# ArmastusChen/Learning-Continuous-Implicit-Representation-for-Near-Periodic-Patterns

Measured on AMD Instinct MI355X. Metric: fitted pixels/sec/GPU (512^2 grid, 256-wide MLP) + iters-to-target-PSNR, higher is better.
Workload: dtype bf16

## Files before the change

learning-continuous-implicit-representation-for-near-periodic-patterns_amd/csrc/npp_api.hip:

```cpp
#include <math.h>
#include <stdarg.h>
#include <stdio.h>
#include <string.h>
#include <vector>

#include "npp_common.h"

namespace npp {

static thread_local char g_err[512] = "";

void set_error(const char* fmt, ...) {
  va_list ap;
  va_start(ap, fmt);
  vsnprintf(g_err, sizeof(g_err), fmt, ap);
  va_end(ap);
}

int check_launch(const char* what) {
  hipError_t e = hipGetLastError();
  if (e != hipSuccess) {
    set_error("%s: %s", what, hipGetErrorString(e));
    return NPP_ERR_LAUNCH;
  }
// ... 190 lines not shown
#pragma unroll
  for (int e = 0; e < 4; ++e) {
    if (e < cnt) {
      if (n < d.n_out[l]) {
        const __bf16 w = (__bf16)pn[e];
        if (!fwd4) {
          const int64_t pf = fwd_pack_pos(d, l, n, k);
          if (pf >= 0) a.wf[pf] = w;
        }
        const int64_t pb = bwd_pack_pos(b, l, n, k);
        if (pb >= 0) a.wb[pb] = w;
      }
      if (++k == d.n_in[l]) { k = 0; ++n; }
      if (n >= d.n_out[l] && i + e + 1 >= d.b_off[l] + d.n_out[l]) {
        do { ++l; } while (l < kNumLayers && !d.present[l]);
        if (l >= kNumLayers) break;
        n = 0; k = 0;
      }
    }
  }
}

static uint16_t f32_to_bf16_host(float f) {
  uint32_t u;
  memcpy(&u, &f, 4);
  if ((u & 0x7fffffffu) > 0x7f800000u) return (uint16_t)((u >> 16) | 0x40);
  u += 0x7FFF + ((u >> 16) & 1);
  return (uint16_t)(u >> 16);
}

__global__ void selftest_kernel(float* out) {
  const int lane = threadIdx.x & 63;
  const int m = lane & 31, h = lane >> 5;
  bf16x8 a, b;
#pragma unroll
  for (int j = 0; j < 8; ++j) {
    const int k = 8 * h + j;
    a[j] = (__bf16)(float)(((m * 3 + k * 5) % 5) - 2);
    b[j] = (__bf16)(float)(((k * 7 + m * 2) % 4) - 1);
  }
  f32x16 acc = {};
  acc = mfma_bf16(a, b, acc);
#pragma unroll
  for (int r = 0; r < 16; ++r) out[acc_row(r, h) * 32 + m] = acc[r];
  f32x16 y = {};
#pragma unroll
  for (int s = 0; s < 2; ++s) {
    bf16x8 x = pack_acc(acc, s), a2;
#pragma unroll
    for (int j = 0; j < 8; ++j) {
      const int k = 16 * s + perm16(h, j);
      a2[j] = (__bf16)(float)(((m * 5 + k * 3) % 7) - 3);
    }
    y = mfma_bf16(a2, x, y);
  }
#pragma unroll
  for (int r = 0; r < 16; ++r) out[1024 + acc_row(r, h) * 32 + m] = y[r];

  __shared__ __attribute__((aligned(16))) char tile[16384];
  for (int u = lane; u < 1024; u += 64) {
    const int hh = u & 1, b = (u >> 1) & 31, bt = (u >> 6) & 1, ks = u >> 7;
    bf16x8 f;
#pragma unroll
    for (int j = 0; j < 8; ++j) {
      const int feat = 16 * ks + perm16(hh, j), row = bt * 32 + b;
      f[j] = (__bf16)(float)(((7 * feat + 3 * row) % 251) - 125);
    }
    *(bf16x8*)(tile + wfmt_unit(8, 0, ks, bt, b, hh)) = f;
  }
  __syncthreads();
  for (int tt = 0; tt < 4; ++tt)
    for (int t = 0; t < 4; ++t) {
      const bf16x8 f = wfrag_read(tile, wfrag_offset(tt, t, lane));
#pragma unroll
      for (int j = 0; j < 8; ++j) out[2048 + ((tt * 4 + t) * 64 + lane) * 8 + j] = (float)f[j];
    }
}

static int tune_env(const char* name, int dflt) {
  const char* e = getenv(name);
  return e && *e ? atoi(e) : dflt;
}
Tunables g_tune = {tune_env("NPP_CONV_WINK", 1), tune_env("NPP_CONV_WIN", 1), tune_env("NPP_CONV_WSTAT", 1), tune_env("NPP_CONV_PAIR", 15),
                   tune_env("NPP_LIGHT_DET", 1), tune_env("NPP_STASH8", 1)};

}

using namespace npp;

extern "C" {

int npp_version(void) { return 100; }

int npp_tune(const char* key, int value) {
  struct { const char* k; int* v; } tab[] = {{"conv_wink", &g_tune.conv_wink}, {"conv_win", &g_tune.conv_win},
                                             {"conv_wstat", &g_tune.conv_wstat}, {"conv_pair", &g_tune.conv_pair},
                                             {"stash8", &g_tune.stash8}, {"light_det", &g_tune.light_det}};
  if (key)
    for (auto& t : tab)
      if (!strcmp(key, t.k)) {
        const int old = __atomic_load_n(t.v, __ATOMIC_RELAXED);
        if (value >= 0) __atomic_store_n(t.v, value, __ATOMIC_RELAXED);
        return old;
      }
  set_error("npp_tune: unknown key '%s'", key ? key : "(null)");
  return NPP_ERR_ARG;
}
const char* npp_last_error_string(void) { return g_err; }

int npp_device_count(void) {
  int n = 0;
  hipError_t e = hipGetDeviceCount(&n);
  if (e != hipSuccess) {
    set_error("hipGetDeviceCount: %s", hipGetErrorString(e));
    (void)hipGetLastError();
    return 0;
  }
  return n;
}

static int check_kw(int K, int width) {
  if (K < 1 || K > NPP_MAX_K) { set_error("K=%d outside [1,%d]", K, NPP_MAX_K); return NPP_ERR_ARG; }
  if (width != NPP_WIDTH) {
    set_error("width=%d: this build is specialised for width %d", width, NPP_WIDTH);
    return NPP_ERR_UNSUPPORTED;
  }
  return NPP_OK;
}

int npp_param_layout(int K, int width, const char** names, int64_t* offsets, int32_t* rows,
                     int32_t* cols, int64_t* total) {
  int rc = check_kw(K, width);
  if (rc) return rc;
  const NetDesc d = make_desc(K);
  int n = 0;
  for (int l = 0; l < kNumLayers; ++l) {
    if (!d.present[l]) continue;
    for (int wb = 0; wb < 2; ++wb) {
      snprintf(g_name_buf[n], sizeof(g_name_buf[n]), "%s.%s", kNames[l], wb ? "bias" : "weight");
      if (names) names[n] = g_name_buf[n];
      if (offsets) offsets[n] = wb ? d.b_off[l] : d.w_off[l];
      if (rows) rows[n] = d.n_out[l];
      if (cols) cols[n] = wb ? 1 : d.n_in[l];
      ++n;
    }
  }
  if (total) *total = d.total_params;
  return n;
}

int64_t npp_pack_bytes(int K, int width, int which) {
  if (check_kw(K, width)) return -1;
  return 16 * (which == 0 ? make_desc(K).wf_total16 : bwd_total16(K));
}

int npp_pack_weights(const float* d_params, void* d_wf, void* d_wb, int K, int width, void* stream) {
  int rc = check_kw(K, width);
  if (rc) return rc;
  if (!d_params || !d_wf || !d_wb) { set_error("npp_pack_weights: null pointer"); return NPP_ERR_ARG; }
  const NetDesc d = make_desc(K);
  const BwdDesc b = make_bwd_desc(K);
  const int64_t nf = d.wf_total16, nb = bwd_total16(K);
  const int threads = 256;
  const int64_t blocks = (nf + nb + threads - 1) / threads;
  hipLaunchKernelGGL(pack_weights_kernel, dim3((unsigned)blocks), dim3(threads), 0, (hipStream_t)stream,
                     d_params, (bf16x8*)d_wf, (bf16x8*)d_wb, d, b, nf, nb);
  return check_launch("npp_pack_weights");
}

int npp_pack_weights_host(const float* params, void* wf, void* wb, int K, int width) {
  int rc = check_kw(K, width);
  if (rc) return rc;
  const NetDesc d = make_desc(K);
  const BwdDesc b = make_bwd_desc(K);
  uint16_t* f = (uint16_t*)wf;
  uint16_t* g = (uint16_t*)wb;
  for (int64_t u = 0; u < d.wf_total16; ++u) {
    int l, ks, nt, lane;
    if (!fwd_unit(d, u, l, ks, nt, lane)) { set_error("fwd unit %lld unmapped", (long long)u); return NPP_ERR_ARG; }
// ... 162 lines not shown
```

learning-continuous-implicit-representation-for-near-periodic-patterns_amd/csrc/npp_common.h:

```cpp
#pragma once
#include <hip/hip_runtime.h>
#include <stdint.h>
#include "npp_layout.h"

typedef __attribute__((ext_vector_type(8))) __bf16 bf16x8;
typedef __attribute__((ext_vector_type(4))) __bf16 bf16x4;
typedef __attribute__((ext_vector_type(2))) __bf16 bf16x2;
typedef __attribute__((ext_vector_type(16))) float f32x16;
typedef __attribute__((ext_vector_type(4))) float f32x4;
typedef __attribute__((ext_vector_type(2))) float f32x2;
typedef __attribute__((ext_vector_type(4))) uint32_t u32x4;
typedef __attribute__((ext_vector_type(8))) _Float16 f16x8;

namespace npp {

void set_error(const char* fmt, ...);
int check_launch(const char* what);
struct SmemOnce { unsigned long long done = 0; };

struct Tunables {
  int conv_wink;
  int conv_win;
  int conv_wstat;
  int conv_pair;
  int light_det;
  int stash8;
};
extern Tunables g_tune;
bool smem_attr(SmemOnce& once, const void* fn, int bytes);

constexpr float kInv2Pi = 0.15915494309189535f;

struct EmbedDev {
  int32_t K, H, W, pad;
  float inv_w, inv_h;
  float cs[NPP_MAX_K][2], sn[NPP_MAX_K][2];
  float per[NPP_MAX_K][2][NPP_N_OFF];
  float freq[NPP_N_FREQ];
  float freq_rev[NPP_N_FREQ];
};

__device__ __forceinline__ float sincos_pi2(float x, bool want_cos) {
  const float jf = rintf(x * 0.636619772367581343f);
  float y = fmaf(-jf, 1.5703125f, x);
  y = fmaf(-jf, 4.837512969970703125e-4f, y);
  y = fmaf(-jf, 7.54978995489188e-8f, y);
  const int q = ((int)jf + (want_cos ? 1 : 0)) & 3;
  const float z = y * y;
  const float s = fmaf(y * z, fmaf(z, fmaf(z, -1.9515295891e-4f, 8.3321608736e-3f), -1.6666654611e-1f), y);
  const float c = fmaf(z * z, fmaf(z, fmaf(z, 2.443315711809948e-5f, -1.388731625493765e-3f), 4.166664568298827e-2f),
                       fmaf(z, -0.5f, 1.0f));
  const float r = (q & 1) ? c : s;
  return (q & 2) ? -r : r;
}

template <bool PRECISE>
__device__ __forceinline__ float warp_value(const EmbedDev& e, int p, int i, float y, float x) {
  const int ori = i >= 11;
  const int ii = ori ? i - 11 : i;
  if (ii == 0) {
    return ori ? (y / (float)e.H - 0.5f) * 2.0f : (x / (float)e.W - 0.5f) * 2.0f;
  }
  const int o = (ii - 1) >> 1;
  const bool is_cos = (ii - 1) & 1;
  const float per = e.per[p][ori][o];
  const float t = __fadd_rn(__fmul_rn(y, e.cs[p][ori]), __fmul_rn(x, e.sn[p][ori]));
  if (PRECISE) {
    float r = fmodf(t, per);
    if (r != 0.0f && ((per < 0.0f) != (r < 0.0f))) r += per;
    const float phi = ((r / per) * 2.0f) * 3.14159265358979323846f;
    return sincos_pi2(phi, is_cos);
  } else {
    const float q = floorf(t / per);
    float r = fmaf(-q, per, t);
    r = r < 0.0f ? r + per : r;
    r = r >= per ? r - per : r;
    const float rev = r / per;
    return is_cos ? __builtin_amdgcn_cosf(rev) : __builtin_amdgcn_sinf(rev);
  }
}

enum CoordMode { kCoordI32 = 0, kCoordF32 = 1, kCoordGrid = 2 };

__device__ __forceinline__ void grid_coord(const npp_grid& g, int64_t r, float& y, float& x) {
  const int64_t p = g.start + (r < g.n ? r : g.n - 1);
  const int64_t i = p / g.width;
  const int32_t j = (int32_t)(p - i * g.width);
  y = __fadd_rn(g.y0, __fdiv_rn((float)i, g.sy));
  x = __fadd_rn(g.x0, __fdiv_rn((float)j, g.sx));
}

template <int CM>
__device__ __forceinline__ void load_coord(const void* coords, const npp_grid& g, int64_t r, float& y, float& x) {
  if (CM == kCoordGrid) {
    grid_coord(g, r, y, x);
  } else if (CM == kCoordF32) {
    const float2 c = ((const float2*)coords)[r];
    y = c.x;
    x = c.y;
  } else {
    const int2 c = ((const int2*)coords)[r];
    y = (float)c.x;
    x = (float)c.y;
  }
}

__device__ __forceinline__ void sincos_pi2_both(float x, float& sn, float& cs) {
  const float jf = rintf(x * 0.636619772367581343f);
  float y = fmaf(-jf, 1.5703125f, x);
// ... 435 lines not shown
```

learning-continuous-implicit-representation-for-near-periodic-patterns_amd/csrc/npp_conv.hip:

```cpp
#include <stdlib.h>
#include <string.h>
#include <type_traits>

#include "npp_common.h"
#include "npp_trunk_layout.h"
#ifdef NPP_DIAG
#include "npp_diag.h"
#else
#define NPP_DIAG_FIELD
#define NPP_DIAG_FILL(a) do { } while (0)
#define NPP_STAMP(a, k) do { } while (0)
#define NPP_STAMP_DRAIN() do { } while (0)
#endif

namespace npp {

#ifndef NPP_CONV_RING
#define NPP_CONV_RING 9
#endif
constexpr int kConvRing = NPP_CONV_RING;
static_assert(kConvRing == 3 || kConvRing == 9, "ring depth");

enum ConvMode : int { kConvFwd = 0, kConvDgradMask = 1, kConvDgradLin = 2, kConvFwdPool = 3, kConvDgradPool = 4 };

// ... 567 lines not shown
    if (has_next) gload(ci + KG, st);
    const char* bA = gbase + buf * kBuf;
    const char* bW = bA + kA + h * wu * 16;
    frag_t A[2][CT], B[2][NPT];
    auto lread = [&](int set, int tap) {
      const int shift = (tap / 3) * a.Wp + (tap % 3);
#pragma unroll
      for (int ct = 0; ct < CT; ++ct) A[set][ct] = *(const frag_t*)(bA + ((ct * 9 + tap) * 64 + lane) * 16);
#pragma unroll
      for (int pt = 0; pt < NPT; ++pt) B[set][pt] = *(const frag_t*)(bW + (posw + 32 * pt + shift) * 16);
    };
    lread(0, 0);
#pragma unroll
    for (int tap = 0; tap < 9; ++tap) {
      if (tap + 1 < 9) lread((tap + 1) & 1, tap + 1);
#pragma unroll
      for (int ct = 0; ct < CT; ++ct)
#pragma unroll
        for (int pt = 0; pt < NPT; ++pt) acc[ct][pt] = mfma16(A[tap & 1][ct], B[tap & 1][pt], acc[ct][pt]);
    }
    if (has_next) sstore(buf ^ 1, st);
    __syncthreads();
    buf ^= 1;
  }
  NPP_STAMP(a, 3);
  float* red = (float*)klds;
  if (KG > 1) {
#pragma unroll
    for (int t = 0; t < NT; ++t) {
      if (t % KG == kg) continue;
#pragma unroll
      for (int r = 0; r < 16; ++r) red[(((pw * KG + kg) * NT + t) * 16 + r) * 64 + lane] = acc[t / NPT][t % NPT][r];
    }
    __syncthreads();
  }
#pragma unroll
  for (int t = 0; t < NT; ++t) {
    if (t % KG != kg) continue;
    const int q = t / KG, ct = t / NPT, pt = t % NPT;
    f32x16 v;
#pragma unroll
    for (int r = 0; r < 16; ++r) v[r] = 0.0f;
#pragma unroll
    for (int g = 0; g < KG; ++g) {
      if (g == kg) {
#pragma unroll
        for (int r = 0; r < 16; ++r) v[r] += acc[ct][pt][r];
      } else {
#pragma unroll
        for (int r = 0; r < 16; ++r) v[r] += red[(((pw * KG + g) * NT + t) * 16 + r) * 64 + lane];
      }
    }
    const int64_t p = (int64_t)(tile0 + NPT * pw + pt) * 32 + b;
    const int n = (int)((uint32_t)p / (uint32_t)a.S);
    const int r0 = (int)(p - (int64_t)n * a.S);
    const int yy = r0 / a.Wp, xx = r0 - yy * a.Wp;
    const bool interior = p < a.npos_valid && yy >= 1 && yy <= a.H && xx >= 1 && xx <= a.W;
    const int64_t tap_base = (((int64_t)n * a.Ctap) * a.H + (yy - 1)) * a.W + (xx - 1);
    const int cot = cot0 + ct;
#pragma unroll
    for (int s = 0; s < 2; ++s) {
      const int chunk = 4 * cot + 2 * s + h;
      if (chunk >= a.cout_chunks) continue;
      const int64_t unit = (int64_t)chunk * a.nposp + kConvGuard + p;
      frag_t o;
#pragma unroll
      for (int j = 0; j < 8; ++j) {
        const int co = 32 * cot + acc_row(8 * s + j, h);
        float x = v[8 * s + j];
        if (FWD) x = fminf(fmaxf(x + bias_r[q][8 * s + j], 0.0f), 65504.0f);
        if (MODE == kConvDgradMask) x = (float)gate[q][s][j] > 0.0f ? x : 0.0f;
        x = interior ? x : 0.0f;
        o[j] = (elem_t)x;
        if (a.tap && interior && co < a.Ctap)
          a.tap[tap_base + (int64_t)co * a.H * a.W] = a.has_scale ? x * a.tap_scale[co & 3] : x;
      }
      if (a.y) ((frag_t*)a.y)[unit] = o;
    }
  }
  NPP_STAMP(a, 4);
  NPP_STAMP_DRAIN();
  NPP_STAMP(a, 5);
  asm volatile("" :: "v"(pf_val));
}

__global__ void conv_pack_kernel(const float* __restrict__ w, int Cin, int Cout, int in_natural, int CIp ,
                                 f16x8* __restrict__ pf, int64_t nf, bf16x8* __restrict__ pb, int64_t nbk) {
  const int64_t u = (int64_t)blockIdx.x * blockDim.x + threadIdx.x;
  if (u < nf) {
    const int lane = (int)(u & 63);
    int64_t r = u >> 6;
    const int tap = (int)(r % 9); r /= 9;
    const int CI = CIp / 16;
    const int ci_step = (int)(r % CI);
    const int cot = (int)(r / CI);
    const int m = lane & 31, h = lane >> 5, co = 32 * cot + m;
    f16x8 o;
#pragma unroll
    for (int j = 0; j < 8; ++j) {
      const int c8 = 2 * ci_step + h;
      const int ci = in_natural ? c8 * 8 + j : conv_chan(c8, j);
      const float v = (co < Cout && ci < Cin) ? w[((int64_t)co * Cin + ci) * 9 + tap] : 0.0f;
      o[j] = (_Float16)fminf(fmaxf(v, -65504.0f), 65504.0f);
    }
    pf[u] = o;
  } else if (u < nf + nbk) {
    const int64_t ub = u - nf;
    const int lane = (int)(ub & 63);
    int64_t r = ub >> 6;
    const int tap = (int)(r % 9); r /= 9;
    const int CO = Cout / 16;
    const int co_step = (int)(r % CO);
    const int cit = (int)(r / CO);
    const int m = lane & 31, h = lane >> 5, ci = 32 * cit + m;
    bf16x8 o;
#pragma unroll
    for (int j = 0; j < 8; ++j) {
      const int co = conv_chan(2 * co_step + h, j);
      const float v = (ci < Cin && co < Cout) ? w[((int64_t)co * Cin + ci) * 9 + (8 - tap)] : 0.0f;
      o[j] = (__bf16)v;
    }
    pb[ub] = o;
  }
}

__global__ void trunk_image_in_kernel(const float* __restrict__ img, int N, int H, int W, float s0, float s1, float s2,
                                      float b0, float b1, float b2, f16x8* __restrict__ out, int64_t nposp,
                                      int64_t npos_round) {
  const int64_t p = (int64_t)blockIdx.x * blockDim.x + threadIdx.x;
  if (p >= npos_round) return;
  const int Wp = W + 2, S = (H + 2) * Wp;
  const int n = (int)(p / S), r = (int)(p - (int64_t)n * S), y = r / Wp, x = r - y * Wp;
  f16x8 o;
#pragma unroll
  for (int j = 0; j < 8; ++j) o[j] = (_Float16)0.0f;
  const f16x8 z = o;
  if (n < N && y >= 1 && y <= H && x >= 1 && x <= W) {
    const int64_t base = ((int64_t)n * 3 * H + (y - 1)) * W + (x - 1);
    const int64_t cs = (int64_t)H * W;
    o[0] = trunk_in_f16(img[base], s0, b0);
    o[1] = trunk_in_f16(img[base + cs], s1, b1);
    o[2] = trunk_in_f16(img[base + 2 * cs], s2, b2);
  }
  out[kConvGuard + p] = o;
  out[nposp + kConvGuard + p] = z;
}

__global__ void trunk_patch_in_kernel(const float* __restrict__ pred, const float* __restrict__ fake,
                                      const float* __restrict__ fmask, const float* __restrict__ real,
                                      const float* __restrict__ rmask, int n_p, int k, int P, int comp, float s0, float s1,
                                      float s2, float b0, float b1, float b2, f16x8* __restrict__ out, int64_t nposp,
                                      int64_t npos_round, float* __restrict__ xy, float* __restrict__ zero, int n_zero,
                                      int which, PixelLossArgs pl, int nb_loss) {
  if ((int)blockIdx.x < nb_loss) {
    pixel_loss_body(pl, (int)blockIdx.x, nb_loss);
    return;
  }
  const int64_t p = (int64_t)((int)blockIdx.x - nb_loss) * blockDim.x + threadIdx.x;
  if (p < n_zero) zero[p] = 0.0f;
  if (p >= npos_round) return;
  const int Wp = P + 2, S = (P + 2) * Wp, nk = n_p * k;
  const int nl = (int)(p / S), r = (int)(p - (int64_t)nl * S), y = r / Wp, x = r - y * Wp;
  const int n_img = which ? nk : 2 * nk;
  const int n = which == 2 ? nl + nk : nl;
  f16x8 o;
#pragma unroll
// ... 333 lines not shown
             (pl->quad == 0.0f && (!pl->latents || !pl->spline || !pl->dlatent || pl->n_knots < 2)))) {
    set_error("%s: bad pixel-loss arguments (N=%lld)", who, (long long)(pl ? pl->N : 0));
    return NPP_ERR_ARG;
  }
  const int64_t nr = conv_npos_round(N, P, P);
  const int nb_loss = pl ? pixel_loss_blocks(pl->N) : 0;
  hipLaunchKernelGGL(trunk_patch_in_kernel, dim3((unsigned)((nr + 255) / 256 + nb_loss)), dim3(256), 0, (hipStream_t)stream,
                     d_pred_rows, d_fake, d_fmask, d_real, d_rmask, n_p, k, P, comp, scale[0], scale[1], scale[2], shift[0], shift[1],
                     shift[2], (f16x8*)d_x0, conv_nposp(N, P, P), nr, d_xy, d_zero, n_zero, which, pl ? *pl : PixelLossArgs{}, nb_loss);
  return check_launch(who);
}

extern "C" int npp_trunk_patch_in(const float* d_pred_rows, const float* d_fake, const float* d_fmask, const float* d_real,
                                  const float* d_rmask, int n_p, int k, int P, int comp, const float scale[3],
                                  const float shift[3], void* d_x0, float* d_xy, float* d_zero, int n_zero, int which,
                                  void* stream) {
  return patch_in_launch(d_pred_rows, d_fake, d_fmask, d_real, d_rmask, n_p, k, P, comp, scale, shift, d_x0, d_xy, d_zero, n_zero,
                         which, nullptr, stream, "npp_trunk_patch_in");
}

extern "C" int npp_trunk_patch_in_loss(const float* d_pred_rows, const float* d_fake, const float* d_fmask, const float* d_real,
                                       const float* d_rmask, int n_p, int k, int P, int comp, const float scale[3],
                                       const float shift[3], void* d_x0, float* d_xy, float* d_zero, int n_zero, int which,
                                       const npp_pixel_loss_args* loss, void* stream) {
  if (!loss) { set_error("npp_trunk_patch_in_loss: null pixel-loss arguments"); return NPP_ERR_ARG; }
  const PixelLossArgs pl{loss->pred, loss->gt, loss->mask, loss->N, loss->latents, loss->spline, loss->n_knots, loss->x_scale,
                         loss->weight, loss->loss, loss->dpred, loss->dlatent, loss->scratch, loss->quad};
  return patch_in_launch(d_pred_rows, d_fake, d_fmask, d_real, d_rmask, n_p, k, P, comp, scale, shift, d_x0, d_xy, d_zero, n_zero,
                         which, &pl, stream, "npp_trunk_patch_in_loss");
}

extern "C" int npp_trunk_patch_in_loss_stack(const float* d_pred, int64_t Bp, int64_t row0, const float* d_crops, int64_t crop_stride,
                                             const float* d_cmasks, int64_t cmask_stride, int M, int n_p, int P, int X, int N_total,
                                             const float scale[3], const float shift[3], void* d_x0, float* d_xy, int64_t xy_stride,
                                             float* d_zero, const void* d_iter, const npp_pixel_loss_args* loss, int64_t gt_stride,
                                             int lat_stride, int loss_stride, int64_t scratch_stride, void* stream) {
  const char* who = "npp_trunk_patch_in_loss_stack";
  if (M < 1 || M > NPP_MAX_STACK || n_p < 1 || X < 0 || 2 * X > N_total || !d_pred || !d_crops || !d_cmasks || !d_x0 || !d_zero ||
      !d_iter || !scale || !shift || !loss || row0 < 0 || row0 + (int64_t)n_p * P * P > Bp) {
    set_error("%s: bad arguments (M=%d n_p=%d X=%d N_total=%d)", who, M, n_p, X, N_total);
    return NPP_ERR_ARG;
  }
  int rc = conv_geom_check(N_total, P, P, who);
  if (rc) return rc;
  if (loss->N <= 0 || !loss->pred || !loss->gt || !loss->loss || !loss->dpred || loss->quad < 0.0f ||
      (loss->quad == 0.0f && (!loss->latents || !loss->spline || !loss->dlatent || loss->n_knots < 2))) {
    set_error("%s: bad pixel-loss arguments (N=%lld)", who, (long long)loss->N);
    return NPP_ERR_ARG;
  }
  PatchInStack a{};
  a.pred = d_pred; a.crops = d_crops; a.cmasks = d_cmasks; a.Bp = Bp; a.row0 = row0; a.crop_stride = crop_stride;
  a.cmask_stride = cmask_stride; a.xy_stride = xy_stride; a.M = M; a.n_p = n_p; a.P = P; a.X = X;
  a.s0 = scale[0]; a.s1 = scale[1]; a.s2 = scale[2]; a.b0 = shift[0]; a.b1 = shift[1]; a.b2 = shift[2];
  a.out = (f16x8*)d_x0; a.nposp = conv_nposp(N_total, P, P);
  a.npos_round = X > 0 ? conv_npos_round(2 * X, P, P) : 0;
  a.xy = d_xy; a.zero = d_zero; a.iter = (const StackIter*)d_iter;
  a.pl = PixelLossArgs{loss->pred, loss->gt, loss->mask, loss->N, loss->latents, loss->spline, loss->n_knots, loss->x_scale,
                       loss->weight, loss->loss, loss->dpred, loss->dlatent, loss->scratch, loss->quad};
  a.gt_stride = gt_stride; a.lat_stride = lat_stride; a.loss_stride = loss_stride; a.scratch_stride = scratch_stride;
  a.nb_loss = pixel_loss_blocks(loss->N);
  const int64_t nblk = (a.npos_round > M ? a.npos_round : M) ;
  hipLaunchKernelGGL(trunk_patch_in_stack_kernel, dim3((unsigned)((nblk + 255) / 256 + (int64_t)M * a.nb_loss)), dim3(256), 0,
                     (hipStream_t)stream, a);
  return check_launch(who);
}

template <int CT, int PT, int S>
static int conv_launch_mode(const ConvArgs& a, int mode, dim3 grid, hipStream_t s) {
  const size_t smem = S > 1 ? (size_t)S * CT * PT * 16 * 64 * sizeof(float) : 0;
#define NPP_CONV_GO(M)                                                                                        \
  do {                                                                                                        \
    static SmemOnce once;                                                                                     \
    if (smem > 48 * 1024 && !smem_attr(once, (const void*)conv3x3_kernel<CT, PT, S, M>, (int)smem)) {          \
      set_error("npp_conv3x3: smem attribute"); return NPP_ERR_LAUNCH;                                        \
    }                                                                                                         \
    hipLaunchKernelGGL((conv3x3_kernel<CT, PT, S, M>), grid, dim3(64 * S), smem, s, a);                       \
  } while (0)
  if (mode == kConvFwd) NPP_CONV_GO(kConvFwd);
  else if (mode == kConvDgradMask) NPP_CONV_GO(kConvDgradMask);
  else if (mode == kConvFwdPool) NPP_CONV_GO(kConvFwdPool);
  else if (mode == kConvDgradPool) NPP_CONV_GO(kConvDgradPool);
  else NPP_CONV_GO(kConvDgradLin);
#undef NPP_CONV_GO
  return NPP_OK;
}

struct PoolFold { const void* x; const void* add; void* dz; void* ypool; };
static int conv3x3_impl(const void* d_x, int N_total, int n_run, int H, int W, int Cin, int Cout, const void* d_pack,
                        const float* d_bias, int mode, const void* d_mask, void* d_y, float* d_tap, int Ctap,
                        const float* tap_scale, const void* d_next_pack, int64_t next_pack_bytes, void* stream,
                        const PoolFold* fold = nullptr);
extern "C" int npp_conv3x3(const void* d_x, int N_total, int n_run, int H, int W, int Cin, int Cout, const void* d_pack,
                           const float* d_bias, int mode, const void* d_mask, void* d_y, float* d_tap, int Ctap,
                           const float* tap_scale, void* stream) {
  return conv3x3_impl(d_x, N_total, n_run, H, W, Cin, Cout, d_pack, d_bias, mode, d_mask, d_y, d_tap, Ctap, tap_scale, nullptr, 0, stream);
}
extern "C" int npp_conv3x3_pf(const void* d_x, int N_total, int n_run, int H, int W, int Cin, int Cout, const void* d_pack,
                              const float* d_bias, int mode, const void* d_mask, void* d_y, float* d_tap, int Ctap,
                              const float* tap_scale, const void* d_next_pack, int64_t next_pack_bytes, void* stream) {
  return conv3x3_impl(d_x, N_total, n_run, H, W, Cin, Cout, d_pack, d_bias, mode, d_mask, d_y, d_tap, Ctap, tap_scale, d_next_pack,
                      next_pack_bytes, stream);
}
extern "C" int npp_conv3x3_dgrad_pool(const void* d_x, int N_total, int n_run, int H, int W, int Cin, int Cout, const void* d_pack,
                                      const void* d_xpre, const void* d_addend, void* d_dz, const void* d_next_pack,
                                      int64_t next_pack_bytes, void* stream) {
  if (!d_xpre || !d_dz) { set_error("npp_conv3x3_dgrad_pool: null pre-pool tensor"); return NPP_ERR_ARG; }
  int rc = conv_geom_check(N_total, 2 * H, 2 * W, "npp_conv3x3_dgrad_pool");
  if (rc) return rc;
  const PoolFold f{d_xpre, d_addend, d_dz, nullptr};
  return conv3x3_impl(d_x, N_total, n_run, H, W, Cin, Cout, d_pack, nullptr, kConvDgradLin, nullptr, d_dz, nullptr, 0, nullptr,
                      d_next_pack, d_next_pack ? next_pack_bytes : 0, stream, &f);
}
extern "C" int npp_conv3x3_pool(const void* d_x, int N_total, int n_run, int H, int W, int Cin, int Cout, const void* d_pack,
                                const float* d_bias, void* d_y, void* d_ypool, float* d_tap, int Ctap, const float* tap_scale,
                                const void* d_next_pack, int64_t next_pack_bytes, void* stream) {
  if (!d_ypool || !d_y || (H & 1) || (W & 1)) { set_error("npp_conv3x3_pool: needs d_y, d_ypool and even H, W (H=%d W=%d)", H, W); return NPP_ERR_ARG; }
  const PoolFold f{nullptr, nullptr, nullptr, d_ypool};
  return conv3x3_impl(d_x, N_total, n_run, H, W, Cin, Cout, d_pack, d_bias, kConvFwd, nullptr, d_y, d_tap, Ctap, tap_scale,
                      d_next_pack, d_next_pack ? next_pack_bytes : 0, stream, &f);
}
static int conv3x3_impl(const void* d_x, int N_total, int n_run, int H, int W, int Cin, int Cout, const void* d_pack,
                        const float* d_bias, int mode, const void* d_mask, void* d_y, float* d_tap, int Ctap,
                        const float* tap_scale, const void* d_next_pack, int64_t next_pack_bytes, void* stream,
                        const PoolFold* fold) {
  int rc = conv_geom_check(N_total, H, W, "npp_conv3x3");
  if (rc) return rc;
  if (!d_x || !d_pack || (!d_y && !d_tap) || mode < 0 || mode > 2 || n_run < 1 || n_run > N_total) {
    set_error("npp_conv3x3: bad argument (mode=%d n_run=%d N=%d)", mode, n_run, N_total);
    return NPP_ERR_ARG;
  }
  if (Cin % 16 || Cout % 16 || Cin < 16 || Cout < 16 || Cin > 512 || Cout > 512) {
    set_error("npp_conv3x3: Cin=%d / Cout=%d must be multiples of 16 in [16, 512] (pad the image to 16 channels)", Cin, Cout);
    return NPP_ERR_ARG;
  }
  if ((mode == kConvFwd && !d_bias) || (mode == kConvDgradMask && !d_mask)) { set_error("npp_conv3x3: mode %d needs bias / mask", mode); return NPP_ERR_ARG; }
  if (d_tap && (Ctap < 1 || Ctap > Cout || (tap_scale && Ctap > 4))) { set_error("npp_conv3x3: bad Ctap=%d", Ctap); return NPP_ERR_ARG; }
  ConvArgs a{};
  a.x = d_x; a.pack = d_pack; a.bias = d_bias; a.mask = d_mask; a.y = d_y; a.tap = d_tap;
  a.N = N_total; a.H = H; a.W = W; a.Wp = W + 2; a.S = (H + 2) * (W + 2); a.CI = Cin / 16; a.cout_chunks = Cout / 8;
  a.Ctap = d_tap ? Ctap : 0; a.has_scale = tap_scale != nullptr;
  for (int i = 0; i < 4; ++i) a.tap_scale[i] = (tap_scale && i < Ctap) ? tap_scale[i] : 1.0f;
  a.nposp = conv_nposp(N_total, H, W);
  a.npos_valid = (int64_t)N_total * a.S;
  const int64_t range = n_run == N_total ? conv_npos_round(N_total, H, W)
                                         : ((int64_t)n_run * a.S + kPosRound - 1) / kPosRound * kPosRound;
  a.pos_tiles = (int)(range / 32);
  a.x_bytes = (uint32_t)((int64_t)(Cin / 8) * a.nposp * 16);
  const int cot_n = (Cout + 31) / 32;
  a.pack_bytes = (uint32_t)((int64_t)cot_n * a.CI * 9 * 1024);
  a.pf = (const char*)d_next_pack;
  a.pf_bytes = d_next_pack ? next_pack_bytes : 0;
  NPP_DIAG_FILL(a);
  if (fold && fold->ypool) {
    a.pool_dz = fold->ypool;
    a.pool_nposp = conv_nposp(N_total, H / 2, W / 2);
    a.pool_cbn = (W + 15) / 16;
    a.pool_tiles = n_run * (H / 2) * a.pool_cbn;
    a.pos_tiles = (a.pool_tiles + 1) / 2 * 2;
    mode = kConvFwdPool;
  } else if (fold) {
    a.pool_x = fold->x; a.pool_add = fold->add; a.pool_dz = fold->dz;
    a.pool_nposp = conv_nposp(N_total, 2 * H, 2 * W);
    a.y = nullptr;
    mode = kConvDgradPool;
  }
  hipStream_t s = (hipStream_t)stream;
  struct Cand { int ct, pt, s; int64_t min_wgs; };
  static const Cand cands[] = {{2, 2, 1, 1024}, {2, 2, 4, 200}, {2, 1, 4, 200}, {1, 1, 4, 100}, {1, 1, 8, 1}, {2, 1, 1, 1}, {1, 1, 1, 1}};
  auto feasible = [&](const Cand& c) { return cot_n % c.ct == 0 && a.CI % c.s == 0 && a.pos_tiles % c.pt == 0; };
  auto wgs = [&](const Cand& c) { return (int64_t)(a.pos_tiles / c.pt) * (cot_n / c.ct); };
  Cand pick = {1, 1, 1, 1};
  static const char* force = getenv("NPP_CONV_TILE");
  bool found = false;
  if (force && strlen(force) == 5 && force[1] == ',' && force[3] == ',') {
    for (const Cand& c : cands)
      if (c.ct == force[0] - '0' && c.pt == force[2] - '0' && c.s == force[4] - '0' && feasible(c)) { pick = c; found = true; }
  }
  const bool forced = found;
  if (!found && a.CI == 1) {
    const Cand c = {2, 1, 1, 1};
    if (feasible(c)) { pick = c; found = true; }
  }
  for (const Cand& c : cands) {
    if (found) break;
    const int64_t need = mode == kConvFwdPool ? c.min_wgs * 9 / 10 : c.min_wgs;
    if (feasible(c) && wgs(c) >= need) { pick = c; found = true; }
  }
  const int wink_mode = __atomic_load_n(&g_tune.conv_wink, __ATOMIC_RELAXED);
  if (wink_mode && !forced && !fold && cot_n % 2 == 0 && a.Wp <= kWinkMaxWp && a.CI % 2 == 0 && (a.CI >= 8 || wink_mode == 2) &&
      (mode == kConvFwd || mode == kConvDgradMask || mode == kConvDgradLin)) {
    const int64_t wgs2 = (int64_t)(a.pos_tiles / 8) * (cot_n / 2), wgs1 = (int64_t)(a.pos_tiles / 4) * (cot_n / 2);
    const int npt = (a.pos_tiles % 8 == 0 && wgs2 >= 200) ? 2 : ((a.pos_tiles % 4 == 0 && (wgs1 >= 200 || wink_mode == 2)) ? 1 : 0);
    if (npt) {
      const int WPk = 128 * npt, wu = (WPk + 2 * (a.Wp + 1) + 7) / 8 * 8;
      const int stage = 2 * 9 * 1024 + 2 * wu * 16;
      const int red = 4 * 2 * (2 * npt) * 4096;
      const int smem = 2 * 2 * stage > red ? 2 * 2 * stage : red;
      const dim3 kgrid((unsigned)(a.pos_tiles / (4 * npt)), (unsigned)(cot_n / 2));
#define NPP_WINK_GO(NPT_, M)                                                                                                    \
      do {                                                                                                                        \
        static SmemOnce once;                                                                                                     \
        if (!smem_attr(once, (const void*)conv3x3_wink_kernel<2, NPT_, 2, M>, 160 * 1024)) { set_error("npp_conv3x3: smem attribute"); return NPP_ERR_LAUNCH; } \
        hipLaunchKernelGGL((conv3x3_wink_kernel<2, NPT_, 2, M>), kgrid, dim3(512), smem, s, a, wu);                               \
      } while (0)
      if (smem <= 160 * 1024) {
        if (npt == 2) { if (mode == kConvFwd) NPP_WINK_GO(2, kConvFwd); else if (mode == kConvDgradMask) NPP_WINK_GO(2, kConvDgradMask); else NPP_WINK_GO(2, kConvDgradLin); }
        else { if (mode == kConvFwd) NPP_WINK_GO(1, kConvFwd); else if (mode == kConvDgradMask) NPP_WINK_GO(1, kConvDgradMask); else NPP_WINK_GO(1, kConvDgradLin); }
        return check_launch("npp_conv3x3");
      }
#undef NPP_WINK_GO
    }
  }
  const int win_mode = __atomic_load_n(&g_tune.conv_win, __ATOMIC_RELAXED);
  const int64_t win_wgs = (int64_t)(a.pos_tiles / 8) * (cot_n / 2);
  if (win_mode && !forced && !fold && a.CI <= 8 && cot_n % 2 == 0 && a.pos_tiles % 8 == 0 && 2 * (a.Wp + 1) + kWinPos <= kWinMaxUnits &&
      ((win_wgs >= 200 && mode == kConvFwd && a.CI <= 4) || win_mode == 2)) {
    const dim3 wgrid((unsigned)(a.pos_tiles / 8), (unsigned)(cot_n / 2));
    constexpr int smem = win_lds_bytes<2>();
#define NPP_WIN_GO(M)                                                                                           \
    do {                                                                                                          \
      static SmemOnce once;                                                                                       \
      if (!smem_attr(once, (const void*)conv3x3_win_kernel<2, M>, smem)) { set_error("npp_conv3x3: smem attribute"); return NPP_ERR_LAUNCH; } \
      hipLaunchKernelGGL((conv3x3_win_kernel<2, M>), wgrid, dim3(256), smem, s, a);                               \
    } while (0)
    if (mode == kConvFwd) NPP_WIN_GO(kConvFwd);
    else if (mode == kConvDgradMask) NPP_WIN_GO(kConvDgradMask);
    else NPP_WIN_GO(kConvDgradLin);
#undef NPP_WIN_GO
    return check_launch("npp_conv3x3");
  }
  dim3 grid((unsigned)(a.pos_tiles / pick.pt), (unsigned)(cot_n / pick.ct));
  const int wstat_mode = __atomic_load_n(&g_tune.conv_wstat, __ATOMIC_RELAXED);
  const int64_t act_bytes = (int64_t)(Cin / 8) * range * 16;
  if (wstat_mode && (int)grid.y >= 8 && (int64_t)a.pack_bytes > 2 * act_bytes) {
    a.wstat = 1; a.wstat_npos = (int)grid.x; a.wstat_ncg = (int)grid.y;
    a.pf = nullptr; a.pf_bytes = 0;
    grid = dim3((unsigned)(8 * (((int)grid.y + 7) / 8) * (int)grid.x), 1);
  }
  int lrc = NPP_OK;
#define NPP_CONV_CASE(CT_, PT_, S_) if (pick.ct == CT_ && pick.pt == PT_ && pick.s == S_) lrc = conv_launch_mode<CT_, PT_, S_>(a, mode, grid, s)
  NPP_CONV_CASE(2, 2, 4); else NPP_CONV_CASE(2, 1, 4); else NPP_CONV_CASE(1, 1, 8); else NPP_CONV_CASE(1, 1, 4);
  else NPP_CONV_CASE(2, 2, 1); else NPP_CONV_CASE(2, 1, 1); else NPP_CONV_CASE(1, 1, 1);
#undef NPP_CONV_CASE
  if (lrc) return lrc;
  return check_launch("npp_conv3x3");
}

extern "C" int npp_maxpool2_fwd(const void* d_x, int N, int H, int W, int C, void* d_y, void* stream) {
  int rc = conv_geom_check(N, H, W, "npp_maxpool2_fwd");
  if (rc) return rc;
  if (!d_x || !d_y || C % 16 || H < 2 || W < 2) { set_error("npp_maxpool2_fwd: bad argument"); return NPP_ERR_ARG; }
  const int64_t nr = conv_npos_round(N, H / 2, W / 2), n = nr * (C / 8);
  hipLaunchKernelGGL(maxpool2_fwd_kernel, dim3((unsigned)((n + 255) / 256)), dim3(256), 0, (hipStream_t)stream, (const f16x8*)d_x,
                     N, H, W, conv_nposp(N, H, W), (f16x8*)d_y, conv_nposp(N, H / 2, W / 2), nr, C / 8);
  return check_launch("npp_maxpool2_fwd");
}

extern "C" int npp_maxpool2_bwd(const void* d_dy, const void* d_x, const void* d_addend, int N_total, int n_run, int H, int W,
                                int C, void* d_dz, void* stream) {
  int rc = conv_geom_check(N_total, H, W, "npp_maxpool2_bwd");
  if (rc) return rc;
  if (!d_dy || !d_x || !d_dz || C % 16 || H < 2 || W < 2 || n_run < 1 || n_run > N_total) { set_error("npp_maxpool2_bwd: bad argument"); return NPP_ERR_ARG; }
  const int64_t S = (int64_t)(H + 2) * (W + 2);
  const int64_t range = n_run == N_total ? conv_npos_round(N_total, H, W) : ((int64_t)n_run * S + kPosRound - 1) / kPosRound * kPosRound;
  const int64_t n = range * (C / 8);
  hipLaunchKernelGGL(maxpool2_bwd_kernel, dim3((unsigned)((n + 255) / 256)), dim3(256), 0, (hipStream_t)stream, (const bf16x8*)d_dy,
                     (const f16x8*)d_x, (const bf16x8*)d_addend, n_run, H, W, conv_nposp(N_total, H, W),
                     conv_nposp(N_total, H / 2, W / 2), range, (bf16x8*)d_dz, C / 8);
  return check_launch("npp_maxpool2_bwd");
}
// ... 46 lines not shown
```

Measured before the change: 46.42 million.

## Add split-K small-spatial conv3x3 kernel for weight-bound deep layers

Adds a specialized 3x3 conv kernel for small spatial sizes where weight bytes dominate activations. Eight waves each take a slice of input channels (split-K), stage their activation windows in LDS, run MFMAs, and reduce partial sums through shared memory. Workgroups are assigned to XCDs explicitly, and a small cost model chooses the half/full output-row split and the tile count. The goal is to spread weight streaming across many CUs on deep low-resolution layers that previously launched too few workgroups. The cost is an extra LDS reduction pass, and prefetch of the next layer's weights is disabled on this path.

```diff
diff --git a/learning-continuous-implicit-representation-for-near-periodic-patterns_amd/csrc/npp_api.hip b/learning-continuous-implicit-representation-for-near-periodic-patterns_amd/csrc/npp_api.hip
--- a/learning-continuous-implicit-representation-for-near-periodic-patterns_amd/csrc/npp_api.hip
+++ b/learning-continuous-implicit-representation-for-near-periodic-patterns_amd/csrc/npp_api.hip
@@ -296,7 +296,7 @@
   return e && *e ? atoi(e) : dflt;
 }
 Tunables g_tune = {tune_env("NPP_CONV_WINK", 1), tune_env("NPP_CONV_WIN", 1), tune_env("NPP_CONV_WSTAT", 1), tune_env("NPP_CONV_PAIR", 15),
-                   tune_env("NPP_LIGHT_DET", 1), tune_env("NPP_STASH8", 1)};
+                   tune_env("NPP_LIGHT_DET", 1), tune_env("NPP_STASH8", 1), tune_env("NPP_CONV_SMALL", 1)};
 
 }
 
@@ -308,7 +308,7 @@
 
 int npp_tune(const char* key, int value) {
   struct { const char* k; int* v; } tab[] = {{"conv_wink", &g_tune.conv_wink}, {"conv_win", &g_tune.conv_win},
-                                             {"conv_wstat", &g_tune.conv_wstat}, {"conv_pair", &g_tune.conv_pair},
+                                             {"conv_wstat", &g_tune.conv_wstat}, {"conv_small", &g_tune.conv_small}, {"conv_pair", &g_tune.conv_pair},
                                              {"stash8", &g_tune.stash8}, {"light_det", &g_tune.light_det}};
   if (key)
     for (auto& t : tab)
diff --git a/learning-continuous-implicit-representation-for-near-periodic-patterns_amd/csrc/npp_common.h b/learning-continuous-implicit-representation-for-near-periodic-patterns_amd/csrc/npp_common.h
--- a/learning-continuous-implicit-representation-for-near-periodic-patterns_amd/csrc/npp_common.h
+++ b/learning-continuous-implicit-representation-for-near-periodic-patterns_amd/csrc/npp_common.h
@@ -25,6 +25,7 @@
   int conv_pair;
   int light_det;
   int stash8;
+  int conv_small;
 };
 extern Tunables g_tune;
 bool smem_attr(SmemOnce& once, const void* fn, int bytes);
diff --git a/learning-continuous-implicit-representation-for-near-periodic-patterns_amd/csrc/npp_conv.hip b/learning-continuous-implicit-representation-for-near-periodic-patterns_amd/csrc/npp_conv.hip
--- a/learning-continuous-implicit-representation-for-near-periodic-patterns_amd/csrc/npp_conv.hip
+++ b/learning-continuous-implicit-representation-for-near-periodic-patterns_amd/csrc/npp_conv.hip
@@ -673,6 +673,189 @@
   NPP_STAMP_DRAIN();
   NPP_STAMP(a, 5);
   asm volatile("" :: "v"(pf_val));
+}
+
+constexpr int kSmS = 8;
+constexpr int kSmMaxWp = 30;
+constexpr int kSmMaxTiles = 32;
+constexpr int kSmCUs = 256;
+template <int PT>
+constexpr int sm_win_units() { return 32 * PT + 2 * (kSmMaxWp + 1); }
+template <bool HALF, int PT>
+constexpr int sm_lds_bytes() {
+  constexpr int win = kSmS * 2 * sm_win_units<PT>() * 16, red = kSmS * PT * (HALF ? 8 : 16) * 256;
+  return win > red ? win : red;
+}
+
+template <bool HALF, int PT, int MODE>
+__global__ __launch_bounds__(64 * kSmS) void conv3x3_small_kernel(ConvArgs a, int ncg , int npg ) {
+  constexpr bool FWD = MODE == kConvFwd, POOLB = MODE == kConvDgradPool;
+  typedef typename OpT<FWD>::frag frag_t;
+  typedef typename OpT<FWD>::elem elem_t;
+  typedef unsigned int u32x4_t __attribute__((ext_vector_type(4)));
+  extern __shared__ __attribute__((aligned(16))) char slds[];
+  const int tid = threadIdx.x, lane = tid & 63;
+  const int wave = __builtin_amdgcn_readfirstlane(tid >> 6);
+  const int b = lane & 31, h = lane >> 5;
+  const int xcd = blockIdx.x & 7, slot = blockIdx.x >> 3;
+  const int cg = xcd + 8 * (slot / npg), pg = slot % npg;
+  if (cg >= ncg) return;
+  const int cot = HALF ? cg >> 1 : cg, rh = HALF ? cg & 1 : 0;
+  const int tile0 = pg * PT;
+  if (a.y && tid < 32 * (HALF ? 2 : 4)) {
+    const int chunk = 4 * cot + 2 * rh + (tid >> 5);
+    if (chunk < a.cout_chunks) {
+      frag_t z;
+#pragma unroll
+      for (int j = 0; j < 8; ++j) z[j] = (elem_t)0.0f;
+      for (int t = npg * PT + pg; t < a.pos_tiles; t += npg)
+        ((frag_t*)a.y)[(int64_t)chunk * a.nposp + kConvGuard + (int64_t)t * 32 + (tid & 31)] = z;
+    }
+  }
+  const int KS = a.CI * 9;
+  const int ci_beg = wave * a.CI / kSmS, ci_end = (wave + 1) * a.CI / kSmS;
+  const wrsrc_t rA = __builtin_amdgcn_make_buffer_rsrc(const_cast<void*>(a.pack), 0, (int)a.pack_bytes, 0x00020000);
+  const wrsrc_t rB = __builtin_amdgcn_make_buffer_rsrc(const_cast<void*>(a.x), 0, (int)a.x_bytes, 0x00020000);
+  const int voffA = (!HALF || ((lane >> 4) & 1) == rh) ? lane * 16 : 0x40000000;
+  const int halo = a.Wp + 1, WIN = 32 * PT + 2 * halo;
+  constexpr int WU = sm_win_units<PT>();
+  constexpr int NW = (2 * WU + 63) / 64;
+  char* const wbase = slds + wave * (2 * WU * 16);
+  int offW[NW], dstW[NW];
+#pragma unroll
+  for (int i = 0; i < NW; ++i) {
+    const int u = lane + 64 * i;
+    const int chunk = u >= WIN, pos = u - chunk * WIN;
+    offW[i] = u < 2 * WIN ? (int)((((int64_t)chunk * a.nposp) + kConvGuard + (int64_t)tile0 * 32 - halo + pos) * 16) : -1;
+    dstW[i] = (chunk * WU + pos) * 16;
+  }
+  frag_t Acur[9], Anxt[9];
+  u32x4_t wreg[NW];
+  auto gloadA = [&](frag_t (&A)[9], int ci) {
+#pragma unroll
+    for (int tap = 0; tap < 9; ++tap)
+      A[tap] = __builtin_bit_cast(frag_t, __builtin_amdgcn_raw_buffer_load_b128(rA, voffA, (int)((uint32_t)(cot * KS + ci * 9 + tap) * 1024u), 0));
+  };
+  auto gloadW = [&](int ci) {
+    const uint32_t soff = (uint32_t)((int64_t)2 * ci * a.nposp * 16);
+#pragma unroll
+    for (int i = 0; i < NW; ++i) wreg[i] = __builtin_amdgcn_raw_buffer_load_b128(rB, offW[i] < 0 ? 0 : offW[i], (int)soff, 0);
+  };
+  f32x16 acc[PT];
+#pragma unroll
+  for (int pt = 0; pt < PT; ++pt)
+#pragma unroll
+    for (int r = 0; r < 16; ++r) acc[pt][r] = 0.0f;
+  constexpr int NS = HALF ? 1 : 2, NU = PT * NS, NR = 8 * NS;
+  static_assert(NU <= kSmS, "one finishing wave per half tile");
+  const bool fin = wave < NU;
+  const int fpt = fin ? wave / NS : 0, fs = HALF ? rh : wave % NS;
+  const int fchunk = 4 * cot + 2 * fs + h;
+  const int64_t fp = (int64_t)(tile0 + fpt) * 32 + b;
+  const bool fdo = fin && fchunk < a.cout_chunks;
+  const int n = (int)((uint32_t)fp / (uint32_t)a.S);
+  const int r0 = (int)(fp - (int64_t)n * a.S);
+  const int yy = r0 / a.Wp, xx = r0 - yy * a.Wp;
+  const bool interior = fp < a.npos_valid && yy >= 1 && yy <= a.H && xx >= 1 && xx <= a.W;
+  f16x8 gate;
+  float bias_r[8];
+  f16x8 pwin[POOLB ? 4 : 1];
+  bf16x8 padd[POOLB ? 4 : 1];
+  const int Wf = 2 * a.W + 2;
+  const int64_t pool_u0 = (int64_t)fchunk * a.pool_nposp + kConvGuard + (int64_t)n * (2 * a.H + 2) * Wf + (int64_t)(2 * yy - 1) * Wf + (2 * xx - 1);
+  if (fdo) {
+    if (MODE == kConvDgradMask) gate = ((const f16x8*)a.mask)[(int64_t)fchunk * a.nposp + kConvGuard + fp];
+    if (FWD) {
+#pragma unroll
+      for (int j = 0; j < 8; ++j) bias_r[j] = a.bias[32 * cot + acc_row(8 * fs + j, h)];
+    }
+    if (POOLB && interior) {
+#pragma unroll
+      for (int k = 0; k < 4; ++k) {
+        const int64_t u = pool_u0 + (k >> 1) * Wf + (k & 1);
+        pwin[k] = ((const f16x8*)a.pool_x)[u];
+        if (a.pool_add) padd[k] = ((const bf16x8*)a.pool_add)[u];
+      }
+    }
+  }
+  if (ci_beg < ci_end) { gloadW(ci_beg); gloadA(Acur, ci_beg); }
+  for (int ci = ci_beg; ci < ci_end; ++ci) {
+#pragma unroll
+    for (int i = 0; i < NW; ++i)
+      if (offW[i] >= 0) *(u32x4_t*)(wbase + dstW[i]) = wreg[i];
+    const bool nx = ci + 1 < ci_end;
+    if (nx) { gloadW(ci + 1); gloadA(Anxt, ci + 1); }
+    asm volatile("s_waitcnt lgkmcnt(0)" ::: "memory");
+    __builtin_amdgcn_wave_barrier();
+    const char* bW = wbase + (h * WU + b) * 16;
+#pragma unroll
+    for (int tap = 0; tap < 9; ++tap) {
+      const int shift = (tap / 3) * a.Wp + (tap % 3);
+#pragma unroll
+      for (int pt = 0; pt < PT; ++pt) acc[pt] = mfma16(Acur[tap], *(const frag_t*)(bW + (32 * pt + shift) * 16), acc[pt]);
+    }
+    asm volatile("" ::: "memory");
+    if (nx) {
+#pragma unroll
+      for (int tap = 0; tap < 9; ++tap) Acur[tap] = Anxt[tap];
+    }
+  }
+  float* const red = (float*)slds;
+  __syncthreads();
+#pragma unroll
+  for (int pt = 0; pt < PT; ++pt)
+#pragma unroll
+    for (int r = 0; r < NR; ++r) {
+      float part;
+      if constexpr (HALF) part = rh ? acc[pt][8 + r] : acc[pt][r];
+      else part = acc[pt][r];
+      red[((wave * PT + pt) * NR + r) * 64 + lane] = part;
+    }
+  __syncthreads();
+  if (!fdo) return;
+  float v[8];
+#pragma unroll
+  for (int j = 0; j < 8; ++j) v[j] = 0.0f;
+  for (int w2 = 0; w2 < kSmS; ++w2)
+#pragma unroll
+    for (int j = 0; j < 8; ++j) v[j] += red[((w2 * PT + fpt) * NR + (HALF ? 0 : 8 * fs) + j) * 64 + lane];
+  if (POOLB) {
+    if (!interior) return;
+    bf16x8 o4[4];
+#pragma unroll
+    for (int j = 0; j < 8; ++j) {
+      const float d = (float)(__bf16)v[j];
+      const float v0 = (float)pwin[0][j], v1 = (float)pwin[1][j], v2 = (float)pwin[2][j], v3 = (float)pwin[3][j];
+      int am = 0;
+      float mx = v0;
+      if (v1 > mx) { mx = v1; am = 1; }
+      if (v2 > mx) { mx = v2; am = 2; }
+      if (v3 > mx) { mx = v3; am = 3; }
+#pragma unroll
+      for (int k = 0; k < 4; ++k) {
+        float g = am == k ? d : 0.0f;
+        if (a.pool_add) g += (float)padd[k][j];
+        o4[k][j] = (__bf16)((float)pwin[k][j] > 0.0f ? g : 0.0f);
+      }
+    }
+#pragma unroll
+    for (int k = 0; k < 4; ++k) ((bf16x8*)a.pool_dz)[pool_u0 + (k >> 1) * Wf + (k & 1)] = o4[k];
+    return;
+  }
+  const int64_t tap_base = (((int64_t)n * a.Ctap) * a.H + (yy - 1)) * a.W + (xx - 1);
+  frag_t o;
+#pragma unroll
+  for (int j = 0; j < 8; ++j) {
+    const int co = 32 * cot + acc_row(8 * fs + j, h);
+    float x = v[j];
+    if (FWD) x = fminf(fmaxf(x + bias_r[j], 0.0f), 65504.0f);
+    if (MODE == kConvDgradMask) x = (float)gate[j] > 0.0f ? x : 0.0f;
+    x = interior ? x : 0.0f;
+    o[j] = (elem_t)x;
+    if (a.tap && interior && co < a.Ctap)
+      a.tap[tap_base + (int64_t)co * a.H * a.W] = a.has_scale ? x * a.tap_scale[co & 3] : x;
+  }
+  if (a.y) ((frag_t*)a.y)[(int64_t)fchunk * a.nposp + kConvGuard + fp] = o;
 }
 
 __global__ void conv_pack_kernel(const float* __restrict__ w, int Cin, int Cout, int in_natural, int CIp ,
@@ -1172,6 +1355,26 @@
   else if (mode == kConvDgradPool) NPP_CONV_GO(kConvDgradPool);
   else NPP_CONV_GO(kConvDgradLin);
 #undef NPP_CONV_GO
+  return NPP_OK;
+}
+
+template <bool HALF, int PT>
+static int conv_small_launch(const ConvArgs& a, int mode, int ncg, int npg, hipStream_t s) {
+  constexpr int smem = sm_lds_bytes<HALF, PT>();
+  const dim3 grid((unsigned)(8 * ((ncg + 7) / 8) * npg));
+#define NPP_SMALL_GO(M)                                                                                       \
+  do {                                                                                                        \
+    static SmemOnce once;                                                                                     \
+    if (smem > 48 * 1024 && !smem_attr(once, (const void*)conv3x3_small_kernel<HALF, PT, M>, smem)) {         \
+      set_error("npp_conv3x3: smem attribute"); return NPP_ERR_LAUNCH;                                        \
+    }                                                                                                         \
+    hipLaunchKernelGGL((conv3x3_small_kernel<HALF, PT, M>), grid, dim3(64 * kSmS), smem, s, a, ncg, npg);     \
+  } while (0)
+  if (mode == kConvFwd) NPP_SMALL_GO(kConvFwd);
+  else if (mode == kConvDgradMask) NPP_SMALL_GO(kConvDgradMask);
+  else if (mode == kConvDgradPool) NPP_SMALL_GO(kConvDgradPool);
+  else NPP_SMALL_GO(kConvDgradLin);
+#undef NPP_SMALL_GO
   return NPP_OK;
 }
 
@@ -1276,6 +1479,36 @@
     const int64_t need = mode == kConvFwdPool ? c.min_wgs * 9 / 10 : c.min_wgs;
     if (feasible(c) && wgs(c) >= need) { pick = c; found = true; }
   }
+  const int small_mode = __atomic_load_n(&g_tune.conv_small, __ATOMIC_RELAXED);
+  const int64_t small_act = (int64_t)(Cin / 8) * (int64_t)a.pos_tiles * 32 * 16;
+  if (small_mode && !forced && mode != kConvFwdPool && a.pos_tiles <= kSmMaxTiles && a.Wp <= kSmMaxWp && cot_n >= 4 &&
+      (int64_t)a.pack_bytes > 2 * small_act) {
+    const int64_t live = a.npos_valid < (int64_t)a.pos_tiles * 32 ? a.npos_valid : (int64_t)a.pos_tiles * 32;
+    const int vt = (int)((live + 31) / 32);
+    int best_h = 1, best_pt = 1;
+    int64_t best = -1;
+    static const char* sforce = getenv("NPP_CONV_SMALL_TILE");
+    if (sforce && strlen(sforce) == 3 && sforce[1] == ',' && (sforce[0] == '0' || sforce[0] == '1') &&
+        (sforce[2] == '1' || sforce[2] == '2' || sforce[2] == '4')) {
+      best_h = sforce[0] - '0'; best_pt = sforce[2] - '0';
+    } else {
+      for (int hf = 1; hf >= 0; --hf)
+        for (int pt = 1; pt <= 4; pt *= 2) {
+          const int64_t wg = (int64_t)cot_n * (hf ? 2 : 1) * ((vt + pt - 1) / pt);
+          const int64_t bytes = (int64_t)a.CI * (9 * (hf ? 512 : 1024) + 2 * (32 * pt + 2 * (a.Wp + 1)) * 16);
+          const int64_t mfma = (int64_t)a.CI * 9 * pt * 8;
+          const int64_t cost = ((wg + kSmCUs - 1) / kSmCUs) * (bytes / 29 + mfma);
+          if (best < 0 || cost < best) { best = cost; best_h = hf; best_pt = pt; }
+        }
+    }
+    const int ncg = cot_n * (best_h ? 2 : 1), npg = (vt + best_pt - 1) / best_pt;
+    a.pf = nullptr; a.pf_bytes = 0;
+    int src = NPP_OK;
+    if (best_h) { if (best_pt == 1) src = conv_small_launch<true, 1>(a, mode, ncg, npg, s); else if (best_pt == 2) src = conv_small_launch<true, 2>(a, mode, ncg, npg, s); else src = conv_small_launch<true, 4>(a, mode, ncg, npg, s); }
+    else { if (best_pt == 1) src = conv_small_launch<false, 1>(a, mode, ncg, npg, s); else if (best_pt == 2) src = conv_small_launch<false, 2>(a, mode, ncg, npg, s); else src = conv_small_launch<false, 4>(a, mode, ncg, npg, s); }
+    if (src) return src;
+    return check_launch("npp_conv3x3");
+  }
   const int wink_mode = __atomic_load_n(&g_tune.conv_wink, __ATOMIC_RELAXED);
   if (wink_mode && !forced && !fold && cot_n % 2 == 0 && a.Wp <= kWinkMaxWp && a.CI % 2 == 0 && (a.CI >= 8 || wink_mode == 2) &&
       (mode == kConvFwd || mode == kConvDgradMask || mode == kConvDgradLin)) {
```

Measured after the change: 46.91 million (median of 6 runs). 1.0% higher.
